# weimengmeng1999/AdapterSIS

Measured on AMD Instinct MI355X. Metric: training images/sec, ViT-L/14 588^2 adapter fine-tune, higher is better.
Workload: dtype f16; 1 GPU; vit_large/14 frozen + CAViT/CACNN adapters (n_last_blocks=4) + FeatureDecoder, 588x588, batch 12/GPU, reference_exact train.py step (fwd + decoder bwd + all-reduce + SGD), random-init weights; global_batch=12, image_size=588, parallelism=dp1, split_precision_convs=True, split_attn_out=False, precise_level=0, fold_attn_scale=True, fused_qkv=False, dead_cacnn_elided=True, c1_elided=True, ln_fold=True, mx_conv=True, mx_dense=True, conv_halo=True, fuse_cls_up=False, skipped_optimizer_steps=0

## Files before the change

adaptersis_amd/csrc/msda.hip:

```cpp
#include "asis_common.h"

namespace {

constexpr int MAX_LP = 16;

template <typename T, int NC = 1>
__global__ __launch_bounds__(256) void msda_fwd_kernel(const T* __restrict__ value, const float* __restrict__ offaw,
                                                       int64_t ld_offaw, const float* __restrict__ ref,
                                                       const int* __restrict__ shapes, const int* __restrict__ starts,
                                                       T* __restrict__ out, T* __restrict__ out_lo, int B, int Lq, int Lin, int M, int L, int P,
                                                       int Dh) {
  const int D = M * Dh;
  const int cpq = D / (8 * NC);
  const int cph = Dh / (8 * NC);
  const int64_t total = (int64_t)B * Lq * cpq;
  const int LP = L * P;
  for (int64_t i = (int64_t)blockIdx.x * blockDim.x + threadIdx.x; i < total; i += (int64_t)gridDim.x * blockDim.x) {
    const int c = (int)(i % cpq);
    const int64_t bq = i / cpq;
    const int q = (int)(bq % Lq);
    const int b = (int)(bq / Lq);
    const int m = c / cph;
    const float* orow = offaw + bq * ld_offaw;
    const float* lg = orow + (int64_t)M * LP * 2 + m * LP;
    float w[MAX_LP];
    float mx = -1e30f;
#pragma unroll
    for (int j = 0; j < MAX_LP; ++j)
      if (j < LP) {
        w[j] = lg[j];
        mx = fmaxf(mx, w[j]);
      }
    float den = 0.f;
#pragma unroll
    for (int j = 0; j < MAX_LP; ++j)
      if (j < LP) {
        w[j] = __expf(w[j] - mx);
        den += w[j];
      }
    const float inv = 1.0f / den;
    const float rx = ref[2 * q], ry = ref[2 * q + 1];
    float acc[8 * NC];
#pragma unroll
    for (int e = 0; e < 8 * NC; ++e) acc[e] = 0.f;
    const T* vb = value + (int64_t)b * Lin * D + c * 8 * NC;
    for (int l = 0; l < L; ++l) {
      const int Hl = shapes[2 * l], Wl = shapes[2 * l + 1];
      const T* vl = vb + (int64_t)starts[l] * D;
#pragma unroll 4
      for (int p = 0; p < P; ++p) {
        const int j = l * P + p;
        const float ox = orow[(m * LP + j) * 2], oy = orow[(m * LP + j) * 2 + 1];
        const float lx = rx + ox / (float)Wl, ly = ry + oy / (float)Hl;
        const float px = lx * (float)Wl - 0.5f, py = ly * (float)Hl - 0.5f;
        const float fx0 = floorf(px), fy0 = floorf(py);
        const float ax = px - fx0, ay = py - fy0;
        const int x0 = (int)fminf(fmaxf(fx0, -2.f), (float)Wl + 1.f);
        const int y0 = (int)fminf(fmaxf(fy0, -2.f), (float)Hl + 1.f);
        const float aw = w[j] * inv;
        uint4 raw[4][NC];
        float wt[4];
#pragma unroll
        for (int t = 0; t < 4; ++t) {
          const int xx = x0 + (t & 1), yy = y0 + (t >> 1);
          const bool inb = (unsigned)xx < (unsigned)Wl && (unsigned)yy < (unsigned)Hl;
          const int xc = xx < 0 ? 0 : (xx >= Wl ? Wl - 1 : xx), yc = yy < 0 ? 0 : (yy >= Hl ? Hl - 1 : yy);
          wt[t] = inb ? ((t & 1) ? ax : 1.f - ax) * ((t >> 1) ? ay : 1.f - ay) * aw : 0.f;
#pragma unroll
          for (int h = 0; h < NC; ++h) raw[t][h] = *reinterpret_cast<const uint4*>(vl + ((int64_t)yc * Wl + xc) * D + 8 * h);
        }
#pragma unroll
        for (int t = 0; t < 4; ++t)
#pragma unroll
          for (int h = 0; h < NC; ++h) {
            float f0, f1;
            unpack2<T>(raw[t][h].x, f0, f1);
            acc[8 * h + 0] += wt[t] * f0; acc[8 * h + 1] += wt[t] * f1;
            unpack2<T>(raw[t][h].y, f0, f1);
            acc[8 * h + 2] += wt[t] * f0; acc[8 * h + 3] += wt[t] * f1;
            unpack2<T>(raw[t][h].z, f0, f1);
            acc[8 * h + 4] += wt[t] * f0; acc[8 * h + 5] += wt[t] * f1;
            unpack2<T>(raw[t][h].w, f0, f1);
            acc[8 * h + 6] += wt[t] * f0; acc[8 * h + 7] += wt[t] * f1;
          }
      }
    }
#pragma unroll
    for (int h = 0; h < NC; ++h) {
      uint4 o;
      o.x = pack2<T>(acc[8 * h + 0], acc[8 * h + 1]);
      o.y = pack2<T>(acc[8 * h + 2], acc[8 * h + 3]);
      o.z = pack2<T>(acc[8 * h + 4], acc[8 * h + 5]);
      o.w = pack2<T>(acc[8 * h + 6], acc[8 * h + 7]);
      *reinterpret_cast<uint4*>(out + bq * D + c * 8 * NC + 8 * h) = o;
      if (out_lo) {
        uint4 ol;
        ol.x = pack2<T>(lo_part<T>(acc[8 * h + 0]), lo_part<T>(acc[8 * h + 1]));
        ol.y = pack2<T>(lo_part<T>(acc[8 * h + 2]), lo_part<T>(acc[8 * h + 3]));
        ol.z = pack2<T>(lo_part<T>(acc[8 * h + 4]), lo_part<T>(acc[8 * h + 5]));
        ol.w = pack2<T>(lo_part<T>(acc[8 * h + 6]), lo_part<T>(acc[8 * h + 7]));
        *reinterpret_cast<uint4*>(out_lo + bq * D + c * 8 * NC + 8 * h) = ol;
      }
    }
  }
}

template <typename T>
__global__ __launch_bounds__(256) void dwconv_gelu_kernel(const float* __restrict__ x, const float* __restrict__ w9,
                                                          const float* __restrict__ bias, const int* __restrict__ shapes,
                                                          const int* __restrict__ starts, int L, T* __restrict__ out,
                                                          int B, int Ntok, int C) {
  const int cpt = C >> 2;
  const int64_t total = (int64_t)B * Ntok * cpt;
  for (int64_t i = (int64_t)blockIdx.x * blockDim.x + threadIdx.x; i < total; i += (int64_t)gridDim.x * blockDim.x) {
    const int c = (int)(i % cpt);
    const int64_t bt = i / cpt;
    const int t = (int)(bt % Ntok);
    const int b = (int)(bt / Ntok);
    int l = 0;
    for (int k = 1; k < L; ++k)
      if (t >= starts[k]) l = k;
    const int Hl = shapes[2 * l], Wl = shapes[2 * l + 1];
    const int p = t - starts[l];
    const int y = p / Wl, xx = p - y * Wl;
    float4 acc = reinterpret_cast<const float4*>(bias)[c];
    const float* xb = x + ((int64_t)b * Ntok + starts[l]) * C;
#pragma unroll
    for (int ky = 0; ky < 3; ++ky)
#pragma unroll
      for (int kx = 0; kx < 3; ++kx) {
        const int yy = y + ky - 1, xs = xx + kx - 1;
        if ((unsigned)yy < (unsigned)Hl && (unsigned)xs < (unsigned)Wl) {
          const float4 v = reinterpret_cast<const float4*>(xb + ((int64_t)yy * Wl + xs) * C)[c];
          const float4 ww = reinterpret_cast<const float4*>(w9 + (ky * 3 + kx) * C)[c];
          acc.x += v.x * ww.x;
          acc.y += v.y * ww.y;
          acc.z += v.z * ww.z;
          acc.w += v.w * ww.w;
        }
      }
    uint2 o;
    o.x = pack2<T>(gelu_erf(acc.x), gelu_erf(acc.y));
    o.y = pack2<T>(gelu_erf(acc.z), gelu_erf(acc.w));
    reinterpret_cast<uint2*>(out + bt * C)[c] = o;
  }
}

}

extern "C" int asis_msda_fwd_split(void* stream, int dtype, const void* value, const float* offaw, int64_t ld_offaw,
                                   const float* ref, const int32_t* shapes, const int32_t* starts, void* out, void* out_lo, int B,
                                   int Lq, int Lin, int M, int L, int P, int Dh) {
  ASIS_REQUIRE(value && offaw && ref && shapes && starts && out, "asis_msda_fwd: null pointer");
  ASIS_REQUIRE(!out_lo || asis_aligned16(out_lo), "asis_msda_fwd_split: out_lo must be 16-byte aligned");
  ASIS_REQUIRE(B > 0 && Lq > 0 && Lin > 0 && M > 0 && L > 0 && P > 0, "asis_msda_fwd: bad shape");
  ASIS_REQUIRE(Dh % 8 == 0, "asis_msda_fwd: head dim %d must be a multiple of 8", Dh);
  ASIS_REQUIRE(L * P <= MAX_LP, "asis_msda_fwd: n_levels*n_points=%d exceeds %d", L * P, MAX_LP);
  ASIS_REQUIRE(ld_offaw >= (int64_t)M * L * P * 3, "asis_msda_fwd: ld_offaw too small");
  ASIS_REQUIRE(asis_aligned16(value) && asis_aligned16(out), "asis_msda_fwd: value/out must be 16-byte aligned");
  ASIS_DT_OK(dtype, "asis_msda_fwd");
  hipStream_t s = reinterpret_cast<hipStream_t>(stream);
  static const int nc_env = [] { const char* e = getenv("ASIS_MSDA_NC"); return e ? atoi(e) : 2; }();
  const int nc = (nc_env >= 2 && Dh % 16 == 0) ? 2 : 1;
  const int64_t total = (int64_t)B * Lq * (M * Dh / (8 * nc));
#define ASIS_MSDA_FWD(NCC)                                                                                        \
  hipLaunchKernelGGL((msda_fwd_kernel<T, NCC>), dim3(asis_grid(total, 256, 1 << 20)), dim3(256), 0, s,             \
                     static_cast<const T*>(value), offaw, ld_offaw, ref, shapes, starts, static_cast<T*>(out),     \
                     static_cast<T*>(out_lo), B, Lq, Lin, M, L, P, Dh)
  if (int rc = asis_dispatch16(dtype, "asis_msda_fwd", [&](auto t) {
        using T = decltype(t);
        if (nc == 2) ASIS_MSDA_FWD(2); else ASIS_MSDA_FWD(1);
      })) return rc;
#undef ASIS_MSDA_FWD
  ASIS_CHECK_LAUNCH("asis_msda_fwd");
  return ASIS_OK;
}

extern "C" int asis_msda_fwd(void* stream, int dtype, const void* value, const float* offaw, int64_t ld_offaw,
                             const float* ref, const int32_t* shapes, const int32_t* starts, void* out, int B, int Lq,
                             int Lin, int M, int L, int P, int Dh) {
  return asis_msda_fwd_split(stream, dtype, value, offaw, ld_offaw, ref, shapes, starts, out, nullptr, B, Lq, Lin, M, L, P, Dh);
}

extern "C" int asis_dwconv_gelu(void* stream, int dtype, const float* x, const float* w9, const float* bias,
                                const int32_t* shapes, const int32_t* starts, int L, void* out, int B, int Ntok,
                                int C) {
  ASIS_REQUIRE(x && w9 && bias && shapes && starts && out, "asis_dwconv_gelu: null pointer");
  ASIS_REQUIRE(C % 4 == 0 && B > 0 && Ntok > 0 && L > 0, "asis_dwconv_gelu: bad shape");
  ASIS_REQUIRE(asis_aligned16(x) && asis_aligned16(w9) && asis_aligned16(bias) && (((uintptr_t)out) & 7) == 0,
               "asis_dwconv_gelu: pointers must be 16-byte aligned");
  ASIS_DT_OK(dtype, "asis_dwconv_gelu");
  const int64_t total = (int64_t)B * Ntok * (C / 4);
  hipStream_t s = reinterpret_cast<hipStream_t>(stream);
  if (int rc = asis_dispatch16(dtype, "asis_dwconv_gelu", [&](auto t) {
        using T = decltype(t);
        hipLaunchKernelGGL((dwconv_gelu_kernel<T>), dim3(asis_grid(total, 256, 256 * 16)), dim3(256), 0, s, x, w9, bias, shapes, starts,
                           L, static_cast<T*>(out), B, Ntok, C);
      })) return rc;
  ASIS_CHECK_LAUNCH("asis_dwconv_gelu");
  return ASIS_OK;
}
```

Baseline: 229.6 img/s.

## Add lean MSDA forward kernel with shared per-point sampling metadata

Adds a new multi-scale deformable attention forward kernel, enabled by default. Each block handles a group of queries and first computes bilinear sample rows, corner weights and softmaxed attention weights once per head/point into LDS. It then gathers 16 channels per thread using packed f16 mixed-precision FMAs. This removes the redundant per-channel-thread recomputation of offsets, softmax and bilinear coordinates in the old kernel. In exchange it adds LDS use, extra barriers and a 32-bit byte-offset addressing limit, and some non-fused multiply-adds mirror the reference rounding.

After: 230.8 img/s (median of 6 runs). No clear change (+0.5%).

```diff
diff --git a/adaptersis_amd/csrc/msda.hip b/adaptersis_amd/csrc/msda.hip
--- a/adaptersis_amd/csrc/msda.hip
+++ b/adaptersis_amd/csrc/msda.hip
@@ -105,6 +105,183 @@
   }
 }
 
+constexpr int LEAN_MAX_ITEMS = 1024;
+
+__device__ __forceinline__ int lean_div(int n, int mg) { return (int)(((unsigned)n * (unsigned)mg) >> 20); }
+static inline int lean_magic(int d) { return ((1 << 20) + d - 1) / d; }
+
+__device__ __forceinline__ float lean_mul_add(float a, float b, float c) {
+#pragma clang fp contract(off)
+  const float p = a * b;
+  return p + c;
+}
+
+template <typename T, bool TWICE> __device__ __forceinline__ void lean_fma8(float (&acc)[16], int h, float wt, const uint4& r) {
+  const uint32_t rw[4] = {r.x, r.y, r.z, r.w};
+#pragma unroll
+  for (int k = 0; k < 4; ++k) {
+    if (TWICE && k == 3) {
+      float f0, f1;
+      unpack2<T>(rw[k], f0, f1);
+      acc[8 * h + 6] = lean_mul_add(wt, f0, acc[8 * h + 6]);
+      acc[8 * h + 7] = lean_mul_add(wt, f1, acc[8 * h + 7]);
+    } else if constexpr (__is_same(T, f16)) {
+      asm("v_fma_mix_f32 %0, %1, %2, %0 op_sel:[0,0,0] op_sel_hi:[0,1,0]" : "+v"(acc[8 * h + 2 * k]) : "v"(wt), "v"(rw[k]));
+      asm("v_fma_mix_f32 %0, %1, %2, %0 op_sel:[0,1,0] op_sel_hi:[0,1,0]" : "+v"(acc[8 * h + 2 * k + 1]) : "v"(wt), "v"(rw[k]));
+    } else {
+      float f0, f1;
+      unpack2<T>(rw[k], f0, f1);
+      acc[8 * h + 2 * k] = __builtin_fmaf(wt, f0, acc[8 * h + 2 * k]);
+      acc[8 * h + 2 * k + 1] = __builtin_fmaf(wt, f1, acc[8 * h + 2 * k + 1]);
+    }
+  }
+}
+
+template <typename T>
+__device__ __forceinline__ void lean_point(float (&acc)[16], const uint4& r, const float4& w, float aw, const char* vb, uint32_t lane_bytes) {
+  const uint32_t row[4] = {r.x, r.y, r.z, r.w};
+  const float wt[4] = {w.x * aw, w.y * aw, w.z * aw, w.w * aw};
+  uint4 raw[4][2];
+#pragma unroll
+  for (int t = 0; t < 4; ++t) {
+    const uint4* p = reinterpret_cast<const uint4*>(vb + (row[t] + lane_bytes));
+    raw[t][0] = p[0];
+    raw[t][1] = p[1];
+  }
+#pragma unroll
+  for (int t = 0; t < 4; ++t) {
+    lean_fma8<T, false>(acc, 0, wt[t], raw[t][0]);
+    if (t == 1 || t == 2) lean_fma8<T, true>(acc, 1, wt[t], raw[t][1]);
+    else lean_fma8<T, false>(acc, 1, wt[t], raw[t][1]);
+  }
+}
+
+template <typename T>
+__global__ __launch_bounds__(256) void msda_fwd_lean_kernel(const T* __restrict__ value, const float* __restrict__ offaw,
+                                                            int64_t ld_offaw, const float* __restrict__ ref,
+                                                            const int* __restrict__ shapes, const int* __restrict__ starts,
+                                                            T* __restrict__ out, T* __restrict__ out_lo, int B, int Lq, int Lin, int M,
+                                                            int L, int P, int Dh, int QB, int mgLP, int mgM, int mgP) {
+  extern __shared__ __attribute__((aligned(16))) unsigned char lean_smem[];
+  const int D = M * Dh;
+  const int cpq = D >> 4;
+  const int cph = Dh >> 4;
+  const int LP = L * P;
+  const int heads = QB * M, items = heads * LP;
+  uint4* s_row = reinterpret_cast<uint4*>(lean_smem);
+  float4* s_wt = reinterpret_cast<float4*>(s_row + items);
+  float* s_aw = reinterpret_cast<float*>(s_wt + items);
+  int* s_lvl = reinterpret_cast<int*>(s_aw + items);
+  const int tid = threadIdx.x;
+  const int BQ = B * Lq;
+  const int groups = (BQ + QB - 1) / QB;
+  const uint32_t row_bytes = (uint32_t)D * (uint32_t)sizeof(T);
+  if (tid < L) {
+    s_lvl[3 * tid] = shapes[2 * tid];
+    s_lvl[3 * tid + 1] = shapes[2 * tid + 1];
+    s_lvl[3 * tid + 2] = starts[tid];
+  }
+  const int gq = tid / cpq, gc = tid - gq * cpq;
+  const int gm = gc / cph;
+  const bool gather = tid < QB * cpq;
+  bool lvl_ready = false;
+  for (int gi = blockIdx.x; gi < groups; gi += gridDim.x) {
+    const int g = (int)gridDim.x == groups ? xcd_remap(gi, groups) : gi;
+    const int bq0 = g * QB;
+    const int b0 = bq0 / Lq;
+    for (int base = 0; base < items; base += 256) {
+      const int it = base + tid;
+      const bool live = it < items;
+      const int hq = lean_div(live ? it : 0, mgLP), qi = lean_div(hq, mgM);
+      const int bq = bq0 + qi;
+      const bool valid = live && bq < BQ;
+      const int b = bq / Lq, q = bq - b * Lq;
+      float lg = 0.f, ox = 0.f, oy = 0.f, rx = 0.f, ry = 0.f;
+      if (valid) {
+        const float* orow = offaw + (int64_t)bq * ld_offaw;
+        const int mj = it - qi * M * LP;
+        lg = orow[M * LP * 2 + mj];
+        ox = orow[mj * 2];
+        oy = orow[mj * 2 + 1];
+        rx = ref[2 * q];
+        ry = ref[2 * q + 1];
+      }
+      if (!lvl_ready) {
+        __syncthreads();
+        lvl_ready = true;
+      }
+      if (!valid) continue;
+      const int j = it - hq * LP, l = lean_div(j, mgP);
+      const int Hl = s_lvl[3 * l], Wl = s_lvl[3 * l + 1], st = s_lvl[3 * l + 2];
+      const float lx = rx + ox / (float)Wl, ly = ry + oy / (float)Hl;
+      const float px = __builtin_fmaf(lx, (float)Wl, -0.5f), py = __builtin_fmaf(ly, (float)Hl, -0.5f);
+      const float fx0 = floorf(px), fy0 = floorf(py);
+      const float ax = px - fx0, ay = py - fy0;
+      const int x0 = (int)fminf(fmaxf(fx0, -2.f), (float)Wl + 1.f);
+      const int y0 = (int)fminf(fmaxf(fy0, -2.f), (float)Hl + 1.f);
+      const int row0 = (b - b0) * Lin + st;
+      uint32_t row[4];
+      float wt[4];
+#pragma unroll
+      for (int t = 0; t < 4; ++t) {
+        const int xx = x0 + (t & 1), yy = y0 + (t >> 1);
+        const bool inb = (unsigned)xx < (unsigned)Wl && (unsigned)yy < (unsigned)Hl;
+        const int xc = xx < 0 ? 0 : (xx >= Wl ? Wl - 1 : xx), yc = yy < 0 ? 0 : (yy >= Hl ? Hl - 1 : yy);
+        wt[t] = inb ? ((t & 1) ? ax : 1.f - ax) * ((t >> 1) ? ay : 1.f - ay) : 0.f;
+        row[t] = (uint32_t)(row0 + yc * Wl + xc) * row_bytes;
+      }
+      s_aw[it] = lg;
+      s_row[it] = make_uint4(row[0], row[1], row[2], row[3]);
+      s_wt[it] = make_float4(wt[0], wt[1], wt[2], wt[3]);
+    }
+    __syncthreads();
+    if (tid < heads && bq0 + lean_div(tid, mgM) < BQ) {
+      float* w = s_aw + tid * LP;
+      float mx = -1e30f;
+      for (int j = 0; j < LP; ++j) mx = fmaxf(mx, w[j]);
+      float den = 0.f;
+      for (int j = 0; j < LP; ++j) {
+        const float e = __expf(w[j] - mx);
+        w[j] = e;
+        den += e;
+      }
+      const float inv = 1.0f / den;
+      for (int j = 0; j < LP; ++j) w[j] = w[j] * inv;
+    }
+    __syncthreads();
+    const int bq = bq0 + gq;
+    if (gather && bq < BQ) {
+      const char* vb = reinterpret_cast<const char*>(value + (int64_t)b0 * Lin * D);
+      const uint32_t lane_bytes = (uint32_t)gc * 16u * (uint32_t)sizeof(T);
+      const int i0 = (gq * M + gm) * LP;
+      float acc[16];
+#pragma unroll
+      for (int e = 0; e < 16; ++e) acc[e] = 0.f;
+#pragma unroll 2
+      for (int j = 0; j < LP; ++j) lean_point<T>(acc, s_row[i0 + j], s_wt[i0 + j], s_aw[i0 + j], vb, lane_bytes);
+      T* po = out + (int64_t)bq * D + gc * 16;
+#pragma unroll
+      for (int h = 0; h < 2; ++h) {
+        uint4 o;
+        o.x = pack2<T>(acc[8 * h + 0], acc[8 * h + 1]);
+        o.y = pack2<T>(acc[8 * h + 2], acc[8 * h + 3]);
+        o.z = pack2<T>(acc[8 * h + 4], acc[8 * h + 5]);
+        o.w = pack2<T>(acc[8 * h + 6], acc[8 * h + 7]);
+        *reinterpret_cast<uint4*>(po + 8 * h) = o;
+        if (out_lo) {
+          uint4 ol;
+          ol.x = pack2<T>(lo_part<T>(acc[8 * h + 0]), lo_part<T>(acc[8 * h + 1]));
+          ol.y = pack2<T>(lo_part<T>(acc[8 * h + 2]), lo_part<T>(acc[8 * h + 3]));
+          ol.z = pack2<T>(lo_part<T>(acc[8 * h + 4]), lo_part<T>(acc[8 * h + 5]));
+          ol.w = pack2<T>(lo_part<T>(acc[8 * h + 6]), lo_part<T>(acc[8 * h + 7]));
+          *reinterpret_cast<uint4*>(out_lo + (int64_t)bq * D + gc * 16 + 8 * h) = ol;
+        }
+      }
+    }
+    if (gi + (int)gridDim.x < groups) __syncthreads();
+  }
+}
+
 template <typename T>
 __global__ __launch_bounds__(256) void dwconv_gelu_kernel(const float* __restrict__ x, const float* __restrict__ w9,
                                                           const float* __restrict__ bias, const int* __restrict__ shapes,
@@ -160,6 +337,30 @@
   ASIS_REQUIRE(asis_aligned16(value) && asis_aligned16(out), "asis_msda_fwd: value/out must be 16-byte aligned");
   ASIS_DT_OK(dtype, "asis_msda_fwd");
   hipStream_t s = reinterpret_cast<hipStream_t>(stream);
+  const char* lean_env = getenv("ASIS_MSDA_LEAN");
+  const int cpq16 = M * Dh / 16;
+  bool lean = !(lean_env && atoi(lean_env) == 0) && Dh % 16 == 0 && cpq16 <= 256 && M * L * P <= LEAN_MAX_ITEMS &&
+              (int64_t)B * Lq < (1ll << 31) - LEAN_MAX_ITEMS;
+  int QB = 0;
+  if (lean) {
+    const int qb_l = 256 / cpq16, qb_i = LEAN_MAX_ITEMS / (M * L * P);
+    QB = qb_l < qb_i ? qb_l : qb_i;
+    const int64_t batches = (QB - 1) / Lq + 2;
+    lean = batches * Lin * M * Dh * 2 < (1ll << 32);
+  }
+  if (lean) {
+    const int items = QB * M * L * P;
+    const size_t lds = (size_t)items * (sizeof(uint4) + sizeof(float4) + sizeof(float)) + (size_t)3 * L * sizeof(int);
+    const int64_t groups = ((int64_t)B * Lq + QB - 1) / QB;
+    if (int rc = asis_dispatch16(dtype, "asis_msda_fwd", [&](auto t) {
+          using T = decltype(t);
+          hipLaunchKernelGGL((msda_fwd_lean_kernel<T>), dim3(asis_grid(groups, 1, 1 << 20)), dim3(256), lds, s,
+                             static_cast<const T*>(value), offaw, ld_offaw, ref, shapes, starts, static_cast<T*>(out),
+                             static_cast<T*>(out_lo), B, Lq, Lin, M, L, P, Dh, QB, lean_magic(L * P), lean_magic(M), lean_magic(P));
+        })) return rc;
+    ASIS_CHECK_LAUNCH("asis_msda_fwd");
+    return ASIS_OK;
+  }
   static const int nc_env = [] { const char* e = getenv("ASIS_MSDA_NC"); return e ? atoi(e) : 2; }();
   const int nc = (nc_env >= 2 && Dh % 16 == 0) ? 2 : 1;
   const int64_t total = (int64_t)B * Lq * (M * Dh / (8 * nc));
```
